# KaranSankla/Lidar_Object_Detection

Measured on AMD Instinct MI355X. Metric: LiDAR points/sec projected+instance-labelled, higher is better.
Workload: dtype f64

## Files before the change

### lidar_object_detection_amd/csrc/lpf_api.hip

```cpp
#include "lpf_kernels.hip.h"
#include "lpf_wide.hip.h"
#include "lpf_cams.hip.h"
#include "lpf_cams_wide.hip.h"
#include "lpf_frame_wide.hip.h"
#include "lpf_depth_maps.hip.h"
#include "lpf_depth_overlays.hip.h"
#include "lpf_match2d.hip.h"
#include "../../include/lpf.h"

#include <algorithm>
#include <cmath>
#include <cstdarg>
#include <cstdio>
#include <cstdlib>
#include <cstring>
#include <dlfcn.h>
#include <mutex>
#include <string>
#include <vector>

#define LPF_SMALL_LAUNCH (7ll << 19)
#define LPF_WIDE_BELOW 480
#define LPF_FEW_BLOCKS 64
#ifndef LPF_TAIL_SPREAD_20THS
#define LPF_TAIL_SPREAD_20THS 13
#endif

#define LPF_RECT_FUSED_TILE 1024

static_assert(sizeof(lpf_frame_summary) == LPF_SUMMARY_BYTES, "summary layout is shared with lpf_finalize_frame");

namespace {

thread_local std::string g_create_error;

struct DevBuf {
    void *p = nullptr;
    size_t cap = 0;
};

}

struct lpf_graph {
    hipGraph_t graph = nullptr;
    hipGraphExec_t exec = nullptr;
    unsigned long long generation = 0;
};

#define LPF_NSETS 4

struct lpf_ctx {
    bool capturing = false;
    unsigned long long generation = 0;
    int device = 0;
    hipStream_t stream = nullptr;
    bool own_stream = false;
    std::string err;

    bool have_camera = false;
    double T[12], K[9], dmin = 0, dmax = 0;
    int W = 0, H = 0;
// ... 174 lines not shown
    const LpfRectJob &GJ = RG ? *RG : norect;
    Y.nrg = RG ? RG->F * RG->bpf : 0;
    Y.nrg8 = (Y.nrg + 7) & ~7;
    Y.ntail = Q.valid ? Q.ntail : 0;
    Y.nk1 = KK.valid ? KK.nk1 : 0;
    Y.npack = 0;
    if (ride) {
        J.masks = (const uint8_t *)c->ride.masks; J.label = c->ride.label; J.M = c->ride.M; J.hw = (long long)c->H * c->W;
        J.rects = c->ride.rects; J.W = c->W;
        J.total16 = (long long)c->ride.F * (J.hw / 16);
        Y.npack = (int)((J.total16 + LPF_BLOCK - 1) / LPF_BLOCK);
    }
    const int nk1_pad = (Y.nk1 + 7) & ~7;
    Y.nper = (Y.ntail + 7) / 8;
    Y.kper = Y.nk1 > 0 ? 8 : 0;
    if (Y.nper > 0 && Y.nk1 > 0) {
        const long long k = ((long long)nk1_pad * LPF_TAIL_SPREAD_20THS / 20 / 8) / Y.nper;
        Y.kper = (int)(k < 1 ? 1 : k) * 8;
    }
    const long long rest = (long long)nk1_pad - (long long)Y.nper * Y.kper;
    Y.rest = (int)(rest > 0 ? rest : 0);
    const long long grid = (long long)Y.nfin8 + Y.nbox8 + Y.nrg8 + (long long)Y.nper * (Y.kper + 8) + Y.rest + Y.npack;
    if (grid > 0) {
        const dim3 gs((unsigned)grid);
        ++c->stats[3];
        if (boxes) ++c->stats[5];
#define LPF_STEP_LAUNCH(RW, LT, PR) do { if (boxes) hipLaunchKernelGGL((lpf_step_t<RW, LPF_K1_FLAGS, LT, PR, true>), gs, dim3(LPF_BLOCK), 0, c->stream, KP, QP, RP, Y, J, XJ, GJ); \
                                         else hipLaunchKernelGGL((lpf_step_t<RW, LPF_K1_FLAGS, LT, PR, false>), gs, dim3(LPF_BLOCK), 0, c->stream, KP, QP, RP, Y, J, XJ, GJ); } while (0)
#define LPF_STEP_LT(RW, PR) do { if (k_lb == 1) LPF_STEP_LAUNCH(RW, uint8_t, PR); else if (k_lb == 2) LPF_STEP_LAUNCH(RW, uint16_t, PR); else LPF_STEP_LAUNCH(RW, uint32_t, PR); } while (0)
        const bool qpre = Q.valid && Q.pre;
        const int rows = KP.tile_pts >> 8;
        if (KK.valid && KK.direct && KK.dsel >= 4) {
            typedef LpfDirectRect<uint8_t, 0> R0; typedef LpfDirectRect<float, 1> R1;
#define LPF_STEP_RECT(RW) do { if (KK.dsel == 4) LPF_STEP_LAUNCH(RW, R0, false); else LPF_STEP_LAUNCH(RW, R1, false); } while (0)
            if (rows == 2) LPF_STEP_RECT(2); else LPF_STEP_RECT(4);
#undef LPF_STEP_RECT
        } else
        if (KK.valid && KK.direct) {
            typedef LpfDirect<uint8_t, 0> D0; typedef LpfDirect<float, 1> D1; typedef LpfDirect<float, 2> D2; typedef LpfDirect<float, 3> D3;
#define LPF_STEP_DIRECT(D) do { if (qpre) LPF_STEP_LAUNCH(2, D, true); else LPF_STEP_LAUNCH(2, D, false); } while (0)
            if (KK.dsel == 0) LPF_STEP_DIRECT(D0); else if (KK.dsel == 1) LPF_STEP_DIRECT(D1); else if (KK.dsel == 2) LPF_STEP_DIRECT(D2); else LPF_STEP_DIRECT(D3);
#undef LPF_STEP_DIRECT
        } else
        if (rows == 2) { if (qpre) LPF_STEP_LT(2, true); else LPF_STEP_LT(2, false); }
        else if (rows == 8) { if (qpre) LPF_STEP_LT(8, true); else LPF_STEP_LT(8, false); }
        else       { if (qpre) LPF_STEP_LT(4, true); else LPF_STEP_LT(4, false); }
#undef LPF_STEP_LT
#undef LPF_STEP_LAUNCH
        LPF_HIP(c, hipGetLastError());
    }
    if (after) LPF_HIP(c, hipEventRecord(after, c->stream));
    if (KK.valid && KK.pre && KK.P.nseg_total > 0) {
        hipLaunchKernelGGL(lpf_scan_segments, dim3(KK.P.F), dim3(LPF_BLOCK), 0, c->stream, KK.P);
        LPF_HIP(c, hipGetLastError());
    }
    return LPF_OK;
}

bool anything_owed(const lpf_ctx *c) { return c->pend_k1.valid || c->pend_tail.valid || c->pend_fin.valid; }

int flush_pending(lpf_ctx *c)
{
    lpf_ctx::BoxSet *XB = &c->bx[c->box_cur];
    if (anything_owed(c)) ++c->stats[1];
    while (anything_owed(c)) {
        const lpf_ctx::Pending K = c->pend_k1, Q = c->pend_tail, R = c->pend_fin;
        int rc_ = launch_step(c, K, Q, R, false, 4, XB, nullptr);
// ... 1027 lines not shown
    NarrowLayout L;
    narrow_layout(c, frame_off, F, BX, out->inst_cap, small, L);
    const bool fused = c->fused && !host_io && pts_on_device && !c->capturing;
    L.split(fused && L.few ? 4 : 1);
    if (c->geometry == 3) L.pre_scan = true;
    if (!fused && anything_owed(c) && (rc = sync_all(c))) return rc;
    lpf_ctx::Scratch &S = c->sc[fused ? c->parity : 0];
    if ((rc = narrow_reserve(c, S, L, M, Btot))) return rc;
    if ((rc = narrow_tables(c, S, L, false))) return rc;
    LpfParams P;
    narrow_params(P, c, ctx_cam(c), L, S, BX, M, out->inst_cap);
    const bool sparse_frames = Ntot * 2 <= (int64_t)F * c->W * c->H;
    const bool direct_rect_fused = c->ride.valid && fused && M > 0 && sparse_frames && !small && c->ride.rects &&
                                   ((!c->ride.f32 && c->ride.mode == 0) || (c->ride.f32 && c->ride.mode == 1));
    const bool direct_fused = direct_rect_fused || (c->ride.valid && fused && small && sparse_frames && M > 0);
    const bool ride_pack = c->ride.valid && fused && !direct_fused && c->ride.can_ride && M > 0;
    if (c->ride.valid && !direct_fused && !ride_pack && (rc = pack_ride_now(c))) return rc;
    const bool direct_rect = M > 0 && c->lazy.valid && !fused && sparse_frames && !small && c->lazy.rects &&
                             ((!c->lazy.f32 && c->lazy.mode == 0) || (c->lazy.f32 && c->lazy.mode == 1));
    const bool direct = direct_rect || (M > 0 && c->lazy.valid && small && sparse_frames && !fused);
    if (M > 0 && c->lazy.valid && !direct && (rc = ensure_packed(c))) return rc;
    const lpf_ctx::Scratch &SM = c->sc[c->mask_set];
    if (M > 0 && fused && !direct && c->mask_set != c->parity)
        return fail(c, LPF_ERR_STATE, "the masks were set for another scratch set: in the pipelined modes the label images rotate with the scratch sets -- call lpf_set_masks_* before every lpf_run* (and after switching modes)");
    P.label_img = (M > 0) ? (direct ? c->lazy.p : direct_fused ? c->ride.masks : SM.label_cur) : nullptr;
    P.rects = (direct && c->lazy.valid) ? c->lazy.rects : (direct_fused && c->ride.valid) ? c->ride.rects : nullptr;
    LpfRectJob RG;
    memset(&RG, 0, sizeof RG);
    const bool rect_tiles = direct_rect || direct_rect_fused;
    if (rect_tiles) {
        RG.rects = P.rects; RG.F = F; RG.M = M;
        RG.cw = (c->W + LPF_RG_CELL - 1) / LPF_RG_CELL; RG.ch = (c->H + LPF_RG_CELL - 1) / LPF_RG_CELL;
        RG.cells = RG.cw * RG.ch; RG.bpf = (RG.cells + LPF_BLOCK - 1) / LPF_BLOCK;
        if ((rc = reserve(c, S.rgrid, (size_t)F * RG.cells * sizeof(uint32_t)))) return rc;
        RG.grid = (uint32_t *)S.rgrid.p;
        P.rect_grid = RG.grid; P.rg_cw = RG.cw; P.rg_cells = RG.cells;
    }
    if (M > 0 && !P.label_img) return fail(c, LPF_ERR_STATE, "no masks for this run's scratch set: in the pipelined modes the label images rotate with the scratch sets -- call lpf_set_masks_* before every lpf_run* (and after switching modes)");

    const size_t n = (size_t)Ntot;
    if (pts_on_device) {
        P.pts = (const float4 *)pts;
    } else {
        if ((rc = reserve(c, c->st_pts, n * 16))) return rc;
        if (n) LPF_HIP(c, hipMemcpyAsync(c->st_pts.p, pts, n * 16, hipMemcpyHostToDevice, c->stream));
        P.pts = (const float4 *)c->st_pts.p;
    }
#define LPF_OUTBUF(field, member, stage, bytes)                                   \
    if (out->member) {                                                            \
        if (host_io) {                                                            \
            if ((rc = reserve(c, c->stage, (bytes)))) return rc;                  \
            P.field = (decltype(P.field))c->stage.p;                              \
        } else {                                                                  \
            P.field = (decltype(P.field))out->member;                             \
        }                                                                         \
    }
    LPF_OUTBUF(uv, uv, st_uv, n * 8)
    LPF_OUTBUF(label_bits, label_bits, st_label, n * 4)
    if (out->uv_valid && !P.uv) { if ((rc = reserve(c, c->st_uv, n * 8))) return rc; P.uv = (decltype(P.uv))c->st_uv.p; }
    if (out->label_valid && !P.label_bits) { if ((rc = reserve(c, c->st_label, n * 4))) return rc; P.label_bits = (decltype(P.label_bits))c->st_label.p; }
    LPF_OUTBUF(uv_valid, uv_valid, st_uvv, n * 8)
    LPF_OUTBUF(label_valid, label_valid, st_labv, n * 4)
    LPF_OUTBUF(depth, depth, st_depth, n * 8)
    LPF_OUTBUF(uf, u_f, st_uf, n * 8)
    LPF_OUTBUF(vf, v_f, st_vf, n * 8)
    LPF_OUTBUF(valid_idx, valid_idx, st_valid, n * 8)
    LPF_OUTBUF(inst_idx, inst_idx, st_inst, (size_t)F * (size_t)out->inst_cap * 8)
    LPF_OUTBUF(count_out, count_mb, st_count, (size_t)(M > 0 ? M : 1) * (Btot > 0 ? Btot : 1) * 4)
    if (host_io || !out->summary) {
// ... 34 lines not shown
            LPF_HIP(c, hipEventCreate(&a));
            LPF_HIP(c, hipEventCreate(&b));
            c->ev.push_back(a); c->ev.push_back(b);
        }
        e0 = c->ev[2 * c->ev_used]; e1 = c->ev[2 * c->ev_used + 1];
        ++c->ev_used;
        LPF_HIP(c, hipEventRecord(e0, c->stream));
    }
    if (fused) {
        lpf_ctx::Pending cur;
        cur.valid = true; cur.P = P; cur.pre = L.pre_scan; cur.ntail = ntail; cur.nk1 = nk1; cur.lb = lb; cur.small = small;
        cur.direct = direct_fused; cur.dsel = direct_rect_fused ? (c->ride.f32 ? 5 : 4) : c->ride.f32 ? c->ride.mode : 0;
        const lpf_ctx::Pending KK = c->defer ? c->pend_k1 : cur, Q = c->pend_tail, R = c->pend_fin;
        if ((rc = launch_step(c, KK, Q, R, ride_pack, lb, &BX, e1, (rect_tiles && c->defer) ? &RG : nullptr))) return rc;
        c->pend_fin = Q;
        c->pend_tail = KK;
        if (c->defer) c->pend_k1 = cur;
        c->ride.valid = false;
        c->parity = (c->parity + 1) % (c->defer ? 4 : 3);
        return LPF_OK;
    }
    if (BX.job_valid && nk1 > 0 && BX.F > 0 && BX.box_off[BX.F] > 0) {
        lpf_ctx::Pending cur, none;
        cur.valid = true; cur.P = P; cur.pre = false; cur.ntail = 0; cur.nk1 = nk1; cur.lb = lb; cur.small = small;
        cur.direct = direct; cur.dsel = direct_rect ? (c->lazy.f32 ? 5 : 4) : c->lazy.f32 ? c->lazy.mode : 0;
        if ((rc = launch_step(c, cur, none, none, false, lb, &BX, e1))) return rc;
    } else {
    if ((rc = launch_box_job(c, BX))) return rc;
    if (nk1 > 0) {
        const dim3 g1((unsigned)nk1);
#define LPF_K1_LAUNCH(R, LT) hipLaunchKernelGGL((lpf_k1_project_t<R, LPF_K1_FLAGS, LT>), g1, dim3(LPF_BLOCK), 0, c->stream, P)
        if (direct_rect) {
            typedef LpfDirectRect<uint8_t, 0> R0; typedef LpfDirectRect<float, 1> R1;
            if (P.tile_pts == 512) { if (!c->lazy.f32) LPF_K1_LAUNCH(2, R0); else LPF_K1_LAUNCH(2, R1); }
            else       { if (!c->lazy.f32) LPF_K1_LAUNCH(4, R0); else LPF_K1_LAUNCH(4, R1); }
        } else if (direct) {
            typedef LpfDirect<uint8_t, 0> D0; typedef LpfDirect<float, 1> D1; typedef LpfDirect<float, 2> D2; typedef LpfDirect<float, 3> D3;
            if (!c->lazy.f32) LPF_K1_LAUNCH(2, D0);
            else if (c->lazy.mode == 1) LPF_K1_LAUNCH(2, D1);
            else if (c->lazy.mode == 2) LPF_K1_LAUNCH(2, D2);
            else LPF_K1_LAUNCH(2, D3);
        } else if (P.tile_pts == 512) { if (lb == 1) LPF_K1_LAUNCH(2, uint8_t); else if (lb == 2) LPF_K1_LAUNCH(2, uint16_t); else LPF_K1_LAUNCH(2, uint32_t); }
        else       { if (lb == 1) LPF_K1_LAUNCH(4, uint8_t); else if (lb == 2) LPF_K1_LAUNCH(4, uint16_t); else LPF_K1_LAUNCH(4, uint32_t); }
#undef LPF_K1_LAUNCH
        LPF_HIP(c, hipGetLastError());
        if (e1) LPF_HIP(c, hipEventRecord(e1, c->stream));
    }
    }
    if (L.pre_scan && L.nseg_total > 0) {
        hipLaunchKernelGGL(lpf_scan_segments, dim3(F), dim3(LPF_BLOCK), 0, c->stream, P);
        LPF_HIP(c, hipGetLastError());
    }
    if (ntail > 0) {
        if (small && P.count_boxes && c->geometry != 4 && (L.nblk <= LPF_WIDE_BELOW || c->geometry == 1)) {
            if (L.pre_scan) hipLaunchKernelGGL((lpf_tail_wide_t<true>), dim3((unsigned)ntail), dim3(64 * LPF_WIDE_WAVES), 0, c->stream, P);
            else hipLaunchKernelGGL((lpf_tail_wide_t<false>), dim3((unsigned)ntail), dim3(64 * LPF_WIDE_WAVES), 0, c->stream, P);
        } else {
            launch_tail(c->stream, P, ntail, L.pre_scan);
        }
        LPF_HIP(c, hipGetLastError());
    }
    hipLaunchKernelGGL(lpf_finalize, dim3(F), dim3(LPF_BLOCK), 0, c->stream, P);
    LPF_HIP(c, hipGetLastError());

    if (host_io) {
        std::vector<lpf_frame_summary> hs((size_t)F);
// ... 1355 lines not shown
```

### lidar_object_detection_amd/csrc/lpf_kernels.hip.h

```cpp
#pragma once
#include <hip/hip_runtime.h>
#include <stdint.h>

#define LPF_BLOCK 256
#define LPF_SEG_QUANTUM 4096
#define LPF_SEG_SMALL 1024
#define LPF_GROUP_SEGS 64
#define LPF_FRM_SHARDS 8
#define LPF_MAX_MASKS_DEV 32
#define LPF_TAB_ROWS 36
#define LPF_TAB_GROUPS 9

struct LpfFrame {
    long long pt_off;
    long long inst_base;
    int N;
    int seg_off;
    int nseg;
    int box_off;
    int B;
    int pad;
    long long cand_off;
    int cand_words;
    int grp_off;
    int shift;
    int pad4;
};

struct LpfParams {
    double T[12];
    double K[9];
    double dmin, dmax;
    int W, H;
    int F, M;
    int seg_pts;
    int nseg_total;
    int nseg_cap;
    int ngrp_cap;
    int oriented;
    long long inst_cap;
    LpfFrame frame0;
    const LpfFrame *frames;
    const LpfFrame *segs;
    const int2 *blks;
    const int4 *cblks;
    int nblk, ncblk;
    int lists_small;
    int csplit;
    const float4 *pts;
    const void *label_img;
    const int4 *rects;
    const uint32_t *rect_grid;
    int rg_cw, rg_cells;
    const double *boxp;
    const float *boxq;
    const unsigned long long *cand;
    int2 *uv;
    uint32_t *label_bits;
    double *depth, *uf, *vf;
    long long *valid_idx;
    int2 *uv_valid;
    uint32_t *label_valid;
    long long *inst_idx;
    int32_t *count_out;
    void *summary;
    unsigned long long *vbal, *mbal;
    uint4 *seg_tab;
    uint4 *grp_tab;
    uint4 *frm_tab;
    uint4 *seg_pre;
    unsigned *cnt;
    float4 *mlist;
    int count_boxes;
    int count_lazy;
    int tile_pts;
};

__device__ __forceinline__ int lpf_lane() { return threadIdx.x & 63; }
__device__ __forceinline__ int lpf_wave() { return threadIdx.x >> 6; }

__device__ __forceinline__ int lpf_xcd_remap(int b, int n)
{
    const int q = n >> 3, r = n & 7, x = b & 7, i = b >> 3;
    return (x < r ? x * (q + 1) : r * (q + 1) + (x - r) * q) + i;
}

// ... 67 lines not shown
                                                      double &uf, double &vf, double &d)
{
    const double x = (double)fx, y = (double)fy, z = (double)fz;
    double cx = TK[0] * x; cx = fma(TK[1], y, cx); cx = fma(TK[2],  z, cx); cx = cx + TK[3];
    double cy = TK[4] * x; cy = fma(TK[5], y, cy); cy = fma(TK[6],  z, cy); cy = cy + TK[7];
    double cz = TK[8] * x; cz = fma(TK[9], y, cz); cz = fma(TK[10], z, cz); cz = cz + TK[11];
    double qx = TK[12] * cx; qx = fma(TK[13], cy, qx); qx = fma(TK[14], cz, qx);
    double qy = TK[15] * cx; qy = fma(TK[16], cy, qy); qy = fma(TK[17], cz, qy);
    d = TK[18] * cx; d = fma(TK[19], cy, d); d = fma(TK[20], cz, d);
    if (d == 0.0) d = -1e-6;
    lpf_div2(qx, qy, fabs(d), uf, vf);
}

__device__ __forceinline__ unsigned lpf_f32_to_u8(float v)
{
    int t;
    if (!(v > -2147483904.0f && v < 2147483648.0f)) t = INT32_MIN; else t = (int)v;
    return (unsigned)t & 0xFFu;
}

template <typename T, int MODE>
__device__ __forceinline__ bool lpf_member(T v)
{
    if (MODE == 0) return v != 0;
    if (MODE == 1) return lpf_f32_to_u8((float)v) != 0u;
    if (MODE == 3) return (float)v > 0.5f;
    return lpf_f32_to_u8((float)v * 255.0f) == 255u;
}

template <typename T, int MODE> struct LpfDirect { };
template <typename LT> struct LpfIsDirect { static constexpr bool value = false; };
template <typename T, int MODE> struct LpfIsDirect<LpfDirect<T, MODE> > { static constexpr bool value = true; };

template <typename T, int MODE> struct LpfDirectRect { };
template <typename LT> struct LpfIsDirectRect { static constexpr bool value = false; };
template <typename T, int MODE> struct LpfIsDirectRect<LpfDirectRect<T, MODE> > { static constexpr bool value = true; };
template <typename T, int MODE> struct LpfIsDirect<LpfDirectRect<T, MODE> > { static constexpr bool value = true; };

template <typename LT>
struct LpfLabelSrc {
    typedef LT elem;
    static __device__ __forceinline__ uint32_t get(const elem *__restrict__ img, const LpfParams &, const int pix, const int4 *, int, int) { return (uint32_t)img[pix]; }
    static __device__ __forceinline__ size_t frame_stride(const LpfParams &P) { return (size_t)P.W * (size_t)P.H; }
};
template <typename T, int MODE>
struct LpfLabelSrc<LpfDirect<T, MODE> > {
    typedef T elem;
    static __device__ __forceinline__ uint32_t get(const elem *__restrict__ msk, const LpfParams &P, const int pix, const int4 *__restrict__ rc,
                                                   const int ui, const int vi)
    {
        const size_t hw = (size_t)P.W * (size_t)P.H;
        uint32_t l = 0;
        for (int m0 = 0; m0 < P.M; m0 += 8) {
            T v[8];
#pragma unroll
            for (int j = 0; j < 8; ++j) v[j] = msk[(size_t)min(m0 + j, P.M - 1) * hw + pix];
#pragma unroll
            for (int j = 0; j < 8; ++j)
                if (m0 + j < P.M && lpf_member<T, MODE>(v[j])) l |= 1u << (m0 + j);
        }
        if (rc && l) {
            uint32_t rest = l;
            while (rest) {
                const int m = __ffs(rest) - 1;
                rest &= rest - 1u;
                const int4 q = rc[m];
                if (!(ui >= q.x && ui < q.z && vi >= q.y && vi < q.w)) l &= ~(1u << m);
            }
        }
        return l;
    }
    static __device__ __forceinline__ size_t frame_stride(const LpfParams &P) { return (size_t)P.M * (size_t)P.W * (size_t)P.H; }
};

template <typename T, int MODE>
struct LpfLabelSrc<LpfDirectRect<T, MODE> > {
    typedef T elem;
    static constexpr int mode = MODE;
    static __device__ __forceinline__ uint32_t get(const elem *__restrict__, const LpfParams &, const int, const int4 *, int, int) { return 0u; }
    static __device__ __forceinline__ size_t frame_stride(const LpfParams &P) { return (size_t)P.M * (size_t)P.W * (size_t)P.H; }
};

#define LPF_F_X4 1u
#define LPF_F_NTLOAD 2u
#define LPF_F_NTSTORE 4u
#define LPF_F_LAB_NOMATH 8u
#define LPF_F_LAB_NOGATHER 16u
#define LPF_F_LAB_NOSTORE 32u

#define LPF_F_LAB_NOBAL 64u
#define LPF_F_LAB_NOTAB 128u

#define LPF_RG_SHIFT 4
#define LPF_RG_CELL (1 << LPF_RG_SHIFT)
__device__ __forceinline__ unsigned lpf_wave_or(unsigned x);

template <int ROWS, unsigned FL, typename LT, bool PRELOADED>
__device__ __forceinline__ void lpf_k1_tile(const LpfParams &P, const int blk, unsigned *s_cnt, float4 (&p)[ROWS])
{
    constexpr int TILE = LPF_BLOCK * ROWS;
    static_assert(LPF_SEG_QUANTUM % TILE == 0 && (LPF_SEG_SMALL % TILE == 0 || ROWS >= 8), "tiles must divide segments (8-row and larger tiles: large geometry only)");
    const int tid = threadIdx.x, lane = lpf_lane(), wave = lpf_wave();
    const int tiles_per_seg = P.seg_pts / TILE;
    const int lb = lpf_xcd_remap(blk, P.nseg_total * tiles_per_seg);
    const int sid = lb / tiles_per_seg;
    LpfFrame fr = P.frame0;
    if (P.F > 1) fr = P.segs[__builtin_amdgcn_readfirstlane(sid)];
    const int f = fr.pad;
    const int sh = fr.shift;
    const long long pbase = fr.pt_off - sh;
    const int seg_start = (sid - fr.seg_off) * P.seg_pts;
    const int seg_end = min(seg_start + P.seg_pts, fr.N + sh);
    const int c = seg_start + (lb - sid * tiles_per_seg) * TILE;
    if (c >= seg_end) return;
    const float4 *__restrict__ pts = P.pts + pbase;
    typedef LpfLabelSrc<LT> Src;
    const typename Src::elem *__restrict__ limg =
        (P.label_img && P.M > 0) ? static_cast<const typename Src::elem *>(P.label_img) + (size_t)f * Src::frame_stride(P) : nullptr;
    const int rows_per_seg = P.seg_pts >> 6;
    if (tid < LPF_TAB_ROWS) s_cnt[tid] = 0;
    __syncthreads();
    unsigned nvalid_w = 0, nmask_w = 0;

    {
        const int wbase = c + wave * (ROWS * 64) + lane;
#pragma unroll
        for (int r = 0; r < ROWS; ++r) {
            if constexpr (PRELOADED) continue;
            const float4 *src = pts + min(wbase + r * 64, seg_end - 1);
            if (FL & LPF_F_NTLOAD) {
                typedef float f4v __attribute__((ext_vector_type(4)));
                const f4v t = __builtin_nontemporal_load(reinterpret_cast<const f4v *>(src));
                p[r] = make_float4(t.x, t.y, t.z, t.w);
            } else {
                p[r] = *src;
            }
        }
        uint32_t lab[ROWS];
        bool valid[ROWS];
        constexpr bool RECT = LpfIsDirectRect<LT>::value;
        const int4 *__restrict__ rc_f = ((RECT || LpfIsDirect<LT>::value) && P.rects) ? P.rects + (size_t)f * P.M : nullptr;
        const uint32_t *__restrict__ rgrid = (RECT && limg && P.rect_grid) ? P.rect_grid + (size_t)f * P.rg_cells : nullptr;
        const size_t mhw = (size_t)P.W * (size_t)P.H;
        unsigned long long myv = 0, mym = 0;
        auto consume = [&](const int r, uint32_t l, const bool okr) {
            const int idx = wbase + r * 64;
            if (idx >= sh && idx < seg_end && P.label_bits && !(FL & LPF_F_LAB_NOSTORE)) {
                if (FL & LPF_F_NTSTORE) __builtin_nontemporal_store(l, P.label_bits + pbase + idx);
                else P.label_bits[pbase + idx] = l;
            }
            const unsigned long long vb = __ballot(okr);
            const unsigned long long mb = __ballot(l != 0);
            if (lane == r) { myv = vb; mym = mb; }
            if (l && P.mlist && !(FL & LPF_F_LAB_NOSTORE))
                P.mlist[pbase + (wbase - lane) + ((wbase - lane) == 0 ? sh : 0) + nmask_w + __popcll(mb & ((1ull << lane) - 1ull))] =
                    make_float4(p[r].x, p[r].y, p[r].z, __uint_as_float(l));
            nvalid_w += __popcll(vb);
            nmask_w += __popcll(mb);
            while (l) {
                const int m = __ffs(l) - 1;
                l &= l - 1;
                atomicAdd(&s_cnt[2 + m], 1u);
            }
        };
#pragma unroll
        for (int r = 0; r < ROWS; ++r) {
            const int idx = wbase + r * 64;
            const bool live = idx >= sh && idx < seg_end;
            if (FL & LPF_F_X4) asm volatile("" ::"v"(p[r].w));
            double uf, vf, d, ru, rv;
            if (FL & LPF_F_LAB_NOMATH) {
                uf = (double)p[r].x; vf = (double)p[r].y; d = (double)p[r].z;
                ru = uf + 700.0; rv = vf + 100.0;
            } else {
                lpf_project_point(P, p[r].x, p[r].y, p[r].z, uf, vf, d);
                ru = rint(uf); rv = rint(vf);
            }
            const int ui = lpf_sat_i32(ru), vi = lpf_sat_i32(rv);
            const bool ok = live && ((unsigned)ui < (unsigned)P.W) && ((unsigned)vi < (unsigned)P.H) &&
                            (d > P.dmin) && (d < P.dmax);
            valid[r] = ok;
            lab[r] = 0;
            if constexpr (RECT) {
                if (ok && rgrid) lab[r] = rgrid[(vi >> LPF_RG_SHIFT) * P.rg_cw + (ui >> LPF_RG_SHIFT)];
            } else
            if (!(FL & LPF_F_LAB_NOGATHER)) {
                if (ok && limg) lab[r] = Src::get(limg, P, vi * P.W + ui, rc_f, ui, vi);
            }
            if (live && !(FL & LPF_F_LAB_NOSTORE)) {
                const long long g = pbase + idx;
                if (P.uv) {
                    if (FL & LPF_F_NTSTORE) {
                        typedef int i2v __attribute__((ext_vector_type(2)));
                        i2v t; t.x = ui; t.y = vi;
                        __builtin_nontemporal_store(t, reinterpret_cast<i2v *>(P.uv + g));
                    } else {
                        P.uv[g] = make_int2(ui, vi);
                    }
                }
                if (P.depth) P.depth[g] = d;
                if (P.uf) P.uf[g] = uf;
                if (P.vf) P.vf[g] = vf;
            }
        }
#pragma unroll
        for (int r = 0; r < ROWS; ++r) {
            uint32_t l = lab[r];
            if constexpr (RECT) {
                if (__any(l != 0u)) {
                    double uf, vf, d;
                    lpf_project_point(P, p[r].x, p[r].y, p[r].z, uf, vf, d);
                    const int ui = lpf_sat_i32(rint(uf)), vi = lpf_sat_i32(rint(vf));
                    const unsigned pix = (unsigned)(vi * P.W + ui);
                    uint32_t any = lpf_wave_or(l), l2 = 0u;
                    while (any) {
                        const int m = __ffs(any) - 1;
                        any &= any - 1u;
                        const int4 q = rc_f[m];
                        const bool in = ((l >> m) & 1u) && ui >= q.x && ui < q.z && vi >= q.y && vi < q.w;
                        if (__any(in)) {
                            const typename Src::elem *__restrict__ mk = limg + (size_t)m * mhw;
                            if (in && lpf_member<typename Src::elem, Src::mode>(mk[pix])) l2 |= 1u << m;
                        }
                    }
                    l = l2;
                }
            }
            consume(r, l, valid[r]);
        }
        if (lane < ROWS && !(FL & LPF_F_LAB_NOBAL)) {
            const size_t row = (size_t)sid * rows_per_seg + ((c - seg_start) >> 6) + wave * ROWS + lane;
            P.vbal[row] = myv;
            P.mbal[row] = mym;
        }
    }
    if (lane == 0) { atomicAdd(&s_cnt[0], nvalid_w); atomicAdd(&s_cnt[1], nmask_w); }
    __syncthreads();
    if (!(FL & LPF_F_LAB_NOTAB)) {
        if (tid < (2 + P.M + 1) >> 1) {
            const unsigned long long v = (unsigned long long)s_cnt[2 * tid] | ((unsigned long long)s_cnt[2 * tid + 1] << 32);
            if (v) {
                int seg_off = P.frame0.seg_off, grp_off = P.frame0.grp_off, fid = P.frame0.pad;
                if (P.F > 1) { const LpfFrame *e = P.segs + lpf_uni(sid); seg_off = e->seg_off; grp_off = e->grp_off; fid = e->pad; }
                const int k = sid - seg_off, g = tid >> 1, h = tid & 1;
                atomicAdd(reinterpret_cast<unsigned long long *>(P.seg_tab + (size_t)g * P.nseg_cap + sid) + h, v);
                atomicAdd(reinterpret_cast<unsigned long long *>(P.grp_tab + (size_t)g * P.ngrp_cap + grp_off + (k >> 6)) + h, v);
                atomicAdd(reinterpret_cast<unsigned long long *>(P.frm_tab + ((size_t)fid * LPF_FRM_SHARDS + (k & (LPF_FRM_SHARDS - 1))) * LPF_TAB_GROUPS + g) + h, v);
            }
        }
    }
}

template <int ROWS, unsigned FL, typename LT>
__device__ __forceinline__ void lpf_k1_tile(const LpfParams &P, const int blk, unsigned *s_cnt)
{
    float4 p[ROWS];
    lpf_k1_tile<ROWS, FL, LT, false>(P, blk, s_cnt, p);
}

template <int ROWS, unsigned FL, typename LT = uint32_t>
__global__ __launch_bounds__(LPF_BLOCK) void lpf_k1_project_t(const LpfParams P)
{
    __shared__ unsigned s_cnt[LPF_TAB_ROWS];
    lpf_k1_tile<ROWS, FL, LT>(P, (int)blockIdx.x, s_cnt);
}

#define LPF_K1_FLAGS (LPF_F_X4 | LPF_F_NTLOAD | LPF_F_NTSTORE)

__device__ __forceinline__ bool lpf_oriented_inside(double px, double py, double pz, const double *__restrict__ b)
{
    const double rx = px - b[0], ry = py - b[1], rz = pz - b[2];
    const bool exact_ok = b[15] != 0.0;
#pragma unroll
    for (int a = 0; a < 3; ++a) {
        const double v0 = b[3 + 4 * a], v1 = b[4 + 4 * a], v2 = b[5 + 4 * a], vv = b[6 + 4 * a];
        double d = v1 * ry; d = fma(v0, rx, d); d = fma(v2, rz, d);
        bool in;
        if (exact_ok && !(fabs(d) < 1e-200 && d != 0.0)) {
            in = (d >= 0.0) && (d <= vv);
        } else {
            const double t = d / vv;
            in = (t >= 0.0) && (t <= 1.0);
        }
        if (!in) return false;
    }
    return true;
}

__device__ __forceinline__ bool lpf_aabb_inside(double px, double py, double pz, const double *__restrict__ b)
{
    return (px >= b[0]) && (px <= b[3]) && (py >= b[1]) && (py <= b[4]) && (pz >= b[2]) && (pz <= b[5]);
}

__device__ __forceinline__ unsigned lpf_rl(unsigned v, int l) { return (unsigned)__builtin_amdgcn_readlane((int)v, l); }
__device__ __forceinline__ float lpf_rlf(float v, int l) { return __int_as_float(__builtin_amdgcn_readlane(__float_as_int(v), l)); }
__device__ __forceinline__ unsigned long long lpf_rl64(unsigned long long v, int l)
{
// ... 636 lines not shown
            w[0] = (long long)tot[0]; w[1] = (long long)tot[1]; w[34] = 0;
            bb[32] = (total > P.inst_cap && P.inst_idx) ? 1 : 0;
            bb[33] = 0;
        }
    }
    if (!staged) {
        __syncthreads();
        for (int i = tid; i < MB; i += LPF_BLOCK) {
            if (out) out[i] = (int32_t)cnt[i];
            cnt[i] = 0;
        }
    }
}

__device__ __forceinline__ int2 lpf_tail_entry(const LpfParams &P, const int i)
{
    if (P.F > 1) return P.blks[i];
    const int first = i * LPF_LISTS_WAVES;
    return make_int2(first, max(0, min(LPF_LISTS_WAVES, P.frame0.nseg - first)));
}
__device__ __forceinline__ void lpf_count_entry(const LpfParams &P, const int i, int &first, int &f, int &nw, int &wd, int &part)
{
    if (P.F > 1) {
        const int4 e = P.cblks[i];
        first = e.x; f = e.y; wd = e.z; nw = e.w & 7; part = e.w >> 3;
        return;
    }
    const int words = max(1, P.frame0.cand_words), per = words * P.csplit;
    const int g = i / per, rem = i - g * per;
    wd = rem / P.csplit; part = rem - wd * P.csplit; f = 0; first = g * LPF_LISTS_WAVES;
    nw = max(0, min(LPF_LISTS_WAVES, P.frame0.nseg - first));
}

struct LpfTailListsLds { unsigned short lidx[LPF_LISTS_WAVES][LPF_LIST_CAP]; };
struct LpfTailCountLds {
    float4 pt[LPF_LISTS_WAVES][64];
    unsigned q[LPF_LISTS_WAVES][128];
    unsigned cnt[LPF_MAX_MASKS_DEV * LPF_BC_WORD / 2];
    float bq[6 * LPF_BC_WORD];
    double bp[LPF_BC_WORD * 16];
    float dom[4];
    unsigned im[LPF_LISTS_WAVES][64], mbase[LPF_LISTS_WAVES][64], L[LPF_LISTS_WAVES];
};

#define LPF_TAIL_LDS (sizeof(LpfTailCountLds) > sizeof(LpfTailListsLds) ? sizeof(LpfTailCountLds) : sizeof(LpfTailListsLds))
#define LPF_STEP_LDS (LPF_TAIL_LDS > sizeof(LpfBoxJobLds) ? LPF_TAIL_LDS : sizeof(LpfBoxJobLds))

template <bool PRE, int STEP>
__device__ __forceinline__ void lpf_tail_block(const LpfParams &P, const int tb, char *s_raw)
{
    LpfTailListsLds &LL = *reinterpret_cast<LpfTailListsLds *>(s_raw);
    LpfTailCountLds &LC = *reinterpret_cast<LpfTailCountLds *>(s_raw);
    const int tid = threadIdx.x, wave = lpf_wave();
    const int ncount = P.count_boxes ? P.ncblk : 0;
    if (tb >= ncount) {
        const int2 ent = lpf_tail_entry(P, tb - ncount);
        const int f = ent.y >> 3, nw = ent.y & 7;
        const LpfFrame fr = lpf_frame_record(P.frame0, P.frames, P.F > 1, f);
        if (wave < nw && (P.valid_idx || P.inst_idx)) {
            if (P.lists_small) lpf_lists_wave_small<PRE>(P, fr, ent.x + wave);
            else lpf_lists_wave<PRE, STEP>(P, fr, ent.x + wave, LL.lidx[wave]);
        }
        return;
    }
    int first, f, nw, wd, part;
    lpf_count_entry(P, tb, first, f, nw, wd, part);
    const LpfFrame fr = lpf_frame_record(P.frame0, P.frames, P.F > 1, f);
    if (wd * LPF_BC_WORD >= fr.B) return;
    if (!P.count_lazy) lpf_count_stage(P, fr, wd, tid, LPF_BLOCK, LC.cnt, LC.bq, LC.bp, LC.dom);
    {
        const int lane = lpf_lane();
        unsigned im = 0, mbase = 0, L = 0;
        if (wave < nw) L = lpf_count_rows(P, fr, first + wave, im, mbase);
        LC.im[wave][lane] = im; LC.mbase[wave][lane] = mbase;
        if (lane == 0) LC.L[wave] = L;
    }
    __syncthreads();
    if (P.count_lazy) {
        if ((LC.L[0] | LC.L[1] | LC.L[2] | LC.L[3]) == 0u) return;
        lpf_count_stage(P, fr, wd, tid, LPF_BLOCK, LC.cnt, LC.bq, LC.bp, LC.dom);
        __syncthreads();
    }
    {
        const int lane = lpf_lane();
        const unsigned L0 = LC.L[0], L1 = LC.L[1], L2 = LC.L[2], L3 = LC.L[3];
        const int c0 = (int)((L0 + 63) >> 6), c1 = (int)((L1 + 63) >> 6), c2 = (int)((L2 + 63) >> 6), c3 = (int)((L3 + 63) >> 6);
        for (int c = part * LPF_LISTS_WAVES + wave; c < c0 + c1 + c2 + c3; c += LPF_LISTS_WAVES * P.csplit) {
            int sg = 0, cc = c;
            if (cc >= c0) { cc -= c0; sg = 1; if (cc >= c1) { cc -= c1; sg = 2; if (cc >= c2) { cc -= c2; sg = 3; } } }
            lpf_count_chunk(P, fr, first + sg, LC.im[sg][lane], LC.mbase[sg][lane], LC.L[sg], (unsigned)cc * 64u, LC.pt[wave], LC.q[wave],
                            LC.cnt, LC.bq, LC.bp, LC.dom, wd);
        }
    }
    __syncthreads();
    lpf_count_flush(P, fr, wd, tid, LPF_BLOCK, LC.cnt);
}

template <bool PRE>
__global__ __launch_bounds__(LPF_BLOCK, 7) void lpf_tail_t(const LpfParams P)
{
// ... 99 lines not shown
    double Tcv[12];
    double K[9];
    int W, H, chunks;
    const LpfBoxFrame *bframes;
    LpfBoxFrame frame0;
    double *boxp; float *boxq; unsigned long long *cand;
    double *corners_keep;
    uint8_t *enabled_out;
    uint8_t *visible; double *corners_out; double *bbox2d; int32_t *front;
};
struct LpfBoxJobLds {
    double c[32][8][3];
    unsigned long long grid[LPF_GRID_CELLS];
    float bnd[64][4];
    float dom[4];
};

__device__ __forceinline__ void lpf_box_frame_block(const LpfBoxJob &J, const int blk, char *s_raw);
struct LpfPackJob {
    const uint8_t *masks;
    void *label;
    long long hw, total16;
    int M, W;
    const int4 *rects;
};
template <typename T, int MODE, typename LT>
__device__ __forceinline__ void lpf_pack16_block(const T *__restrict__ masks, LT *__restrict__ label,
                                                 const int M, const long long hw, const long long total16, const long long blk,
                                                 const int4 *__restrict__ rects, const int W);

struct LpfRectJob {
    const int4 *rects;
    uint32_t *grid;
    int F, M, cw, ch, cells, bpf;
};
__device__ __forceinline__ void lpf_rect_grid_block(const LpfRectJob &G, const int blk)
{
    const int f = blk / G.bpf, i = (blk - f * G.bpf) * LPF_BLOCK + (int)threadIdx.x;
    if (f >= G.F || i >= G.cells) return;
    const int cy = i / G.cw, cx = i - cy * G.cw;
    const int x0 = cx << LPF_RG_SHIFT, y0 = cy << LPF_RG_SHIFT;
    const int4 *__restrict__ rc = G.rects + (size_t)lpf_uni(f) * G.M;
    uint32_t bits = 0u;
    for (int m0 = 0; m0 < G.M; m0 += 8) {
        int4 q[8];
#pragma unroll
        for (int j = 0; j < 8; ++j) q[j] = rc[min(m0 + j, G.M - 1)];
#pragma unroll
        for (int j = 0; j < 8; ++j)
            if (m0 + j < G.M && q[j].x < x0 + LPF_RG_CELL && q[j].z > x0 && q[j].y < y0 + LPF_RG_CELL && q[j].w > y0 && q[j].z > q[j].x && q[j].w > q[j].y)
                bits |= 1u << (m0 + j);
    }
    G.grid[(size_t)f * G.cells + i] = bits;
}
__global__ __launch_bounds__(LPF_BLOCK) void lpf_rect_grid_kernel(const LpfRectJob G) { lpf_rect_grid_block(G, (int)blockIdx.x); }

template <int ROWS, unsigned FL, typename LT, bool PRE, bool BOXES>
__global__ __launch_bounds__(LPF_BLOCK, 7) void lpf_step_t(const LpfParams P, const LpfParams Q, const LpfParams R, const LpfStepLayout Y,
                                                           const LpfPackJob J, const LpfBoxJob X, const LpfRectJob G)
{
    __shared__ __attribute__((aligned(16))) char s_raw[LPF_STEP_LDS];
    __shared__ unsigned s_cnt[LPF_TAB_ROWS];
    int b = (int)blockIdx.x;
    LPF_ROLE_BEGIN
    if (b < Y.nfin8) {
        if (b < Y.nfin) {
            const LpfFrame fr = lpf_frame_record(R.frame0, R.frames, R.F > 1, b);
            lpf_finalize_frame(R, fr, b, s_cnt, reinterpret_cast<unsigned *>(s_raw));
            LPF_ROLE_END(0)
        }
        return;
    }
    b -= Y.nfin8;
    if (b < Y.nbox8) {
        if constexpr (BOXES) {
            if (b < Y.nbox) { lpf_box_frame_block(X, b, s_raw); LPF_ROLE_END(1) }
        }
        return;
    }
    b -= Y.nbox8;
    if (b < Y.nrg8) {
        if (b < Y.nrg) lpf_rect_grid_block(G, b);
        return;
    }
    b -= Y.nrg8;
    const int plen = Y.kper + 8, periodic = Y.nper * plen;
    int vblk;
    if (b < periodic) {
        const int per = b / plen, pos = b - per * plen;
        if (pos >= Y.kper) {
            const int tb = per * 8 + (pos - Y.kper);
            if (tb < Y.ntail) { lpf_tail_block<PRE, 2>(Q, tb, s_raw); LPF_ROLE_END(tb < (Q.count_boxes ? Q.ncblk : 0) ? 3 : 2) }
            return;
        }
        vblk = ((per * (Y.kper >> 3) + (pos >> 3)) << 3) | (pos & 7);
    } else {
        const int r = b - periodic;
        if (r >= Y.rest) {
            if constexpr (!LpfIsDirect<LT>::value) {
                if (r - Y.rest < Y.npack) { lpf_pack16_block<uint8_t, 0, LT>(J.masks, static_cast<LT *>(J.label), J.M, J.hw, J.total16, r - Y.rest, J.rects, J.W); LPF_ROLE_END(4) }
            }
            return;
        }
        vblk = ((Y.nper * (Y.kper >> 3) + (r >> 3)) << 3) | (r & 7);
    }
    const int x = vblk & 7, q = Y.nk1 >> 3, rem = Y.nk1 & 7;
    if ((vblk >> 3) >= q + (x < rem ? 1 : 0)) return;
    lpf_k1_tile<ROWS, FL, LT>(P, vblk, s_cnt);
    LPF_ROLE_END(5)
}

__global__ __launch_bounds__(LPF_BLOCK) void lpf_resize_linear_u8_kernel(const uint8_t *__restrict__ src, uint8_t *__restrict__ dst,
                                                                         const int4 *__restrict__ xtab, const int4 *__restrict__ ytab,
                                                                         const int w, const int h, const int W, const int H, const long long total)
{
    const long long i = (long long)blockIdx.x * LPF_BLOCK + threadIdx.x;
    if (i >= total) return;
    const long long hw = (long long)W * H;
    const long long n = i / hw;
    const int rem = (int)(i - n * hw), y = rem / W, x = rem - y * W;
    const int4 cx = xtab[x], cy = ytab[y];
    const uint8_t *__restrict__ s = src + (size_t)n * w * h;
    const int r0 = cy.x * w, r1 = cy.y * w;
    const int S0 = (int)s[r0 + cx.x] * cx.z + (int)s[r0 + cx.y] * cx.w;
    const int S1 = (int)s[r1 + cx.x] * cx.z + (int)s[r1 + cx.y] * cx.w;
    dst[i] = (uint8_t)((((cy.z * (S0 >> 4)) >> 16) + ((cy.w * (S1 >> 4)) >> 16) + 2) >> 2);
}

#define LPF_R2H_BLOCKS 8
struct LpfToHost {
    long long *valid_idx; int2 *uv_valid; uint32_t *label_valid; long long *inst_idx; int32_t *count_mb; void *summary;
    long long inst_cap;
    int n_count;
};

__global__ __launch_bounds__(LPF_BLOCK) void lpf_results_to_host(const LpfParams P, const LpfToHost D)
{
    const int f = (int)blockIdx.x / LPF_R2H_BLOCKS, part = (int)blockIdx.x - f * LPF_R2H_BLOCKS;
    if (f >= P.F) return;
    const LpfFrame fr = lpf_frame_record(P.frame0, P.frames, P.F > 1, f);
    const long long *S = reinterpret_cast<const long long *>(static_cast<const char *>(P.summary) + (size_t)f * LPF_SUMMARY_BYTES);
// ... 526 lines not shown
```

Before: 173.1 billion.

## Add LDS cell-occupancy bitmap to skip rect-grid gathers; early-exit empty count blocks

```diff
diff --git a/lidar_object_detection_amd/csrc/lpf_api.hip b/lidar_object_detection_amd/csrc/lpf_api.hip
--- a/lidar_object_detection_amd/csrc/lpf_api.hip
+++ b/lidar_object_detection_amd/csrc/lpf_api.hip
@@ -27,6 +27,9 @@
 #endif
 
 #define LPF_RECT_FUSED_TILE 1024
+#ifndef LPF_RECT_LDS
+#define LPF_RECT_LDS 1
+#endif
 
 static_assert(sizeof(lpf_frame_summary) == LPF_SUMMARY_BYTES, "summary layout is shared with lpf_finalize_frame");
 
@@ -267,7 +270,9 @@
         const int rows = KP.tile_pts >> 8;
         if (KK.valid && KK.direct && KK.dsel >= 4) {
             typedef LpfDirectRect<uint8_t, 0> R0; typedef LpfDirectRect<float, 1> R1;
-#define LPF_STEP_RECT(RW) do { if (KK.dsel == 4) LPF_STEP_LAUNCH(RW, R0, false); else LPF_STEP_LAUNCH(RW, R1, false); } while (0)
+            typedef LpfDirectRect<uint8_t, 0, true> R0L; typedef LpfDirectRect<float, 1, true> R1L;
+#define LPF_STEP_RECT(RW) do { if (KP.rg_lds) { if (KK.dsel == 4) LPF_STEP_LAUNCH(RW, R0L, false); else LPF_STEP_LAUNCH(RW, R1L, false); } \
+                               else { if (KK.dsel == 4) LPF_STEP_LAUNCH(RW, R0, false); else LPF_STEP_LAUNCH(RW, R1, false); } } while (0)
             if (rows == 2) LPF_STEP_RECT(2); else LPF_STEP_RECT(4);
 #undef LPF_STEP_RECT
         } else
@@ -1361,9 +1366,14 @@
         RG.rects = P.rects; RG.F = F; RG.M = M;
         RG.cw = (c->W + LPF_RG_CELL - 1) / LPF_RG_CELL; RG.ch = (c->H + LPF_RG_CELL - 1) / LPF_RG_CELL;
         RG.cells = RG.cw * RG.ch; RG.bpf = (RG.cells + LPF_BLOCK - 1) / LPF_BLOCK;
-        if ((rc = reserve(c, S.rgrid, (size_t)F * RG.cells * sizeof(uint32_t)))) return rc;
+        RG.occ_words = (RG.cells + 63) / 64;
+        const size_t grid_bytes = ((size_t)F * RG.cells * sizeof(uint32_t) + 7) & ~(size_t)7;
+        if ((rc = reserve(c, S.rgrid, grid_bytes + (size_t)F * RG.occ_words * sizeof(unsigned long long)))) return rc;
         RG.grid = (uint32_t *)S.rgrid.p;
+        RG.occ = (unsigned long long *)((char *)S.rgrid.p + grid_bytes);
         P.rect_grid = RG.grid; P.rg_cw = RG.cw; P.rg_cells = RG.cells;
+        P.rect_occ = RG.occ; P.rg_occ_words = RG.occ_words;
+        P.rg_lds = (LPF_RECT_LDS && RG.occ_words <= LPF_RG_LDS_WORDS) ? 1 : 0;
     }
     if (M > 0 && !P.label_img) return fail(c, LPF_ERR_STATE, "no masks for this run's scratch set: in the pipelined modes the label images rotate with the scratch sets -- call lpf_set_masks_* before every lpf_run* (and after switching modes)");
 
@@ -1464,6 +1474,11 @@
 #define LPF_K1_LAUNCH(R, LT) hipLaunchKernelGGL((lpf_k1_project_t<R, LPF_K1_FLAGS, LT>), g1, dim3(LPF_BLOCK), 0, c->stream, P)
         if (direct_rect) {
             typedef LpfDirectRect<uint8_t, 0> R0; typedef LpfDirectRect<float, 1> R1;
+            typedef LpfDirectRect<uint8_t, 0, true> R0L; typedef LpfDirectRect<float, 1, true> R1L;
+            if (P.rg_lds) {
+                if (P.tile_pts == 512) { if (!c->lazy.f32) LPF_K1_LAUNCH(2, R0L); else LPF_K1_LAUNCH(2, R1L); }
+                else       { if (!c->lazy.f32) LPF_K1_LAUNCH(4, R0L); else LPF_K1_LAUNCH(4, R1L); }
+            } else
             if (P.tile_pts == 512) { if (!c->lazy.f32) LPF_K1_LAUNCH(2, R0); else LPF_K1_LAUNCH(2, R1); }
             else       { if (!c->lazy.f32) LPF_K1_LAUNCH(4, R0); else LPF_K1_LAUNCH(4, R1); }
         } else if (direct) {
diff --git a/lidar_object_detection_amd/csrc/lpf_kernels.hip.h b/lidar_object_detection_amd/csrc/lpf_kernels.hip.h
--- a/lidar_object_detection_amd/csrc/lpf_kernels.hip.h
+++ b/lidar_object_detection_amd/csrc/lpf_kernels.hip.h
@@ -52,6 +52,9 @@
     const int4 *rects;
     const uint32_t *rect_grid;
     int rg_cw, rg_cells;
+    const unsigned long long *rect_occ;
+    int rg_occ_words;
+    int rg_lds;
     const double *boxp;
     const float *boxq;
     const unsigned long long *cand;
@@ -185,10 +188,10 @@
 template <typename LT> struct LpfIsDirect { static constexpr bool value = false; };
 template <typename T, int MODE> struct LpfIsDirect<LpfDirect<T, MODE> > { static constexpr bool value = true; };
 
-template <typename T, int MODE> struct LpfDirectRect { };
-template <typename LT> struct LpfIsDirectRect { static constexpr bool value = false; };
-template <typename T, int MODE> struct LpfIsDirectRect<LpfDirectRect<T, MODE> > { static constexpr bool value = true; };
-template <typename T, int MODE> struct LpfIsDirect<LpfDirectRect<T, MODE> > { static constexpr bool value = true; };
+template <typename T, int MODE, bool GRID_LDS = false> struct LpfDirectRect { };
+template <typename LT> struct LpfIsDirectRect { static constexpr bool value = false; static constexpr bool grid_lds = false; };
+template <typename T, int MODE, bool G> struct LpfIsDirectRect<LpfDirectRect<T, MODE, G> > { static constexpr bool value = true; static constexpr bool grid_lds = G; };
+template <typename T, int MODE, bool G> struct LpfIsDirect<LpfDirectRect<T, MODE, G> > { static constexpr bool value = true; };
 
 template <typename LT>
 struct LpfLabelSrc {
@@ -226,8 +229,8 @@
     static __device__ __forceinline__ size_t frame_stride(const LpfParams &P) { return (size_t)P.M * (size_t)P.W * (size_t)P.H; }
 };
 
-template <typename T, int MODE>
-struct LpfLabelSrc<LpfDirectRect<T, MODE> > {
+template <typename T, int MODE, bool G>
+struct LpfLabelSrc<LpfDirectRect<T, MODE, G> > {
     typedef T elem;
     static constexpr int mode = MODE;
     static __device__ __forceinline__ uint32_t get(const elem *__restrict__, const LpfParams &, const int, const int4 *, int, int) { return 0u; }
@@ -246,10 +249,11 @@
 
 #define LPF_RG_SHIFT 4
 #define LPF_RG_CELL (1 << LPF_RG_SHIFT)
+#define LPF_RG_LDS_WORDS 512
 __device__ __forceinline__ unsigned lpf_wave_or(unsigned x);
 
 template <int ROWS, unsigned FL, typename LT, bool PRELOADED>
-__device__ __forceinline__ void lpf_k1_tile(const LpfParams &P, const int blk, unsigned *s_cnt, float4 (&p)[ROWS])
+__device__ __forceinline__ void lpf_k1_tile(const LpfParams &P, const int blk, unsigned *s_cnt, float4 (&p)[ROWS], unsigned long long *s_occ = nullptr)
 {
     constexpr int TILE = LPF_BLOCK * ROWS;
     static_assert(LPF_SEG_QUANTUM % TILE == 0 && (LPF_SEG_SMALL % TILE == 0 || ROWS >= 8), "tiles must divide segments (8-row and larger tiles: large geometry only)");
@@ -271,8 +275,10 @@
     const typename Src::elem *__restrict__ limg =
         (P.label_img && P.M > 0) ? static_cast<const typename Src::elem *>(P.label_img) + (size_t)f * Src::frame_stride(P) : nullptr;
     const int rows_per_seg = P.seg_pts >> 6;
+    constexpr bool RECT = LpfIsDirectRect<LT>::value;
+    constexpr bool grid_lds = LpfIsDirectRect<LT>::grid_lds;
     if (tid < LPF_TAB_ROWS) s_cnt[tid] = 0;
-    __syncthreads();
+    if constexpr (!grid_lds) __syncthreads();
     unsigned nvalid_w = 0, nmask_w = 0;
 
     {
@@ -291,7 +297,18 @@
         }
         uint32_t lab[ROWS];
         bool valid[ROWS];
-        constexpr bool RECT = LpfIsDirectRect<LT>::value;
+        const bool have_grid = RECT && limg && P.rect_grid;
+        if constexpr (grid_lds) {
+            unsigned long long t[LPF_RG_LDS_WORDS / LPF_BLOCK];
+            const unsigned long long *__restrict__ occ = P.rect_occ + (size_t)f * P.rg_occ_words;
+#pragma unroll
+            for (int k = 0; k < LPF_RG_LDS_WORDS / LPF_BLOCK; ++k)
+                t[k] = (have_grid && k * LPF_BLOCK + tid < P.rg_occ_words) ? occ[k * LPF_BLOCK + tid] : 0ull;
+#pragma unroll
+            for (int k = 0; k < LPF_RG_LDS_WORDS / LPF_BLOCK; ++k)
+                if (k * LPF_BLOCK < P.rg_occ_words) s_occ[k * LPF_BLOCK + tid] = t[k];
+            __syncthreads();
+        }
         const int4 *__restrict__ rc_f = ((RECT || LpfIsDirect<LT>::value) && P.rects) ? P.rects + (size_t)f * P.M : nullptr;
         const uint32_t *__restrict__ rgrid = (RECT && limg && P.rect_grid) ? P.rect_grid + (size_t)f * P.rg_cells : nullptr;
         const size_t mhw = (size_t)P.W * (size_t)P.H;
@@ -316,6 +333,21 @@
                 atomicAdd(&s_cnt[2 + m], 1u);
             }
         };
+        auto rect_exact = [&](const uint32_t l, const int ui, const int vi) -> uint32_t {
+            const unsigned pix = (unsigned)(vi * P.W + ui);
+            uint32_t any = lpf_wave_or(l), l2 = 0u;
+            while (any) {
+                const int m = __ffs(any) - 1;
+                any &= any - 1u;
+                const int4 q = rc_f[m];
+                const bool in = ((l >> m) & 1u) && ui >= q.x && ui < q.z && vi >= q.y && vi < q.w;
+                if (__any(in)) {
+                    const typename Src::elem *__restrict__ mk = limg + (size_t)m * mhw;
+                    if constexpr (RECT) { if (in && lpf_member<typename Src::elem, Src::mode>(mk[pix])) l2 |= 1u << m; }
+                }
+            }
+            return l2;
+        };
 #pragma unroll
         for (int r = 0; r < ROWS; ++r) {
             const int idx = wbase + r * 64;
@@ -335,7 +367,7 @@
             valid[r] = ok;
             lab[r] = 0;
             if constexpr (RECT) {
-                if (ok && rgrid) lab[r] = rgrid[(vi >> LPF_RG_SHIFT) * P.rg_cw + (ui >> LPF_RG_SHIFT)];
+                if constexpr (!grid_lds) { if (ok && rgrid) lab[r] = rgrid[(vi >> LPF_RG_SHIFT) * P.rg_cw + (ui >> LPF_RG_SHIFT)]; }
             } else
             if (!(FL & LPF_F_LAB_NOGATHER)) {
                 if (ok && limg) lab[r] = Src::get(limg, P, vi * P.W + ui, rc_f, ui, vi);
@@ -355,28 +387,26 @@
                 if (P.uf) P.uf[g] = uf;
                 if (P.vf) P.vf[g] = vf;
             }
+            if constexpr (grid_lds) {
+                const int cell = ok ? (vi >> LPF_RG_SHIFT) * P.rg_cw + (ui >> LPF_RG_SHIFT) : 0;
+                const bool cand = ok && ((s_occ[cell >> 6] >> (cell & 63)) & 1ull);
+                uint32_t l = 0u;
+                if (__any(cand)) {
+                    if (cand) l = rgrid[cell];
+                    if (__any(l != 0u)) l = rect_exact(l, ui, vi);
+                }
+                consume(r, l, ok);
+            }
         }
 #pragma unroll
         for (int r = 0; r < ROWS; ++r) {
+            if constexpr (grid_lds) break;
             uint32_t l = lab[r];
             if constexpr (RECT) {
                 if (__any(l != 0u)) {
                     double uf, vf, d;
                     lpf_project_point(P, p[r].x, p[r].y, p[r].z, uf, vf, d);
-                    const int ui = lpf_sat_i32(rint(uf)), vi = lpf_sat_i32(rint(vf));
-                    const unsigned pix = (unsigned)(vi * P.W + ui);
-                    uint32_t any = lpf_wave_or(l), l2 = 0u;
-                    while (any) {
-                        const int m = __ffs(any) - 1;
-                        any &= any - 1u;
-                        const int4 q = rc_f[m];
-                        const bool in = ((l >> m) & 1u) && ui >= q.x && ui < q.z && vi >= q.y && vi < q.w;
-                        if (__any(in)) {
-                            const typename Src::elem *__restrict__ mk = limg + (size_t)m * mhw;
-                            if (in && lpf_member<typename Src::elem, Src::mode>(mk[pix])) l2 |= 1u << m;
-                        }
-                    }
-                    l = l2;
+                    l = rect_exact(l, lpf_sat_i32(rint(uf)), lpf_sat_i32(rint(vf)));
                 }
             }
             consume(r, l, valid[r]);
@@ -405,17 +435,22 @@
 }
 
 template <int ROWS, unsigned FL, typename LT>
-__device__ __forceinline__ void lpf_k1_tile(const LpfParams &P, const int blk, unsigned *s_cnt)
+__device__ __forceinline__ void lpf_k1_tile(const LpfParams &P, const int blk, unsigned *s_cnt, unsigned long long *s_occ = nullptr)
 {
     float4 p[ROWS];
-    lpf_k1_tile<ROWS, FL, LT, false>(P, blk, s_cnt, p);
+    lpf_k1_tile<ROWS, FL, LT, false>(P, blk, s_cnt, p, s_occ);
 }
 
 template <int ROWS, unsigned FL, typename LT = uint32_t>
 __global__ __launch_bounds__(LPF_BLOCK) void lpf_k1_project_t(const LpfParams P)
 {
     __shared__ unsigned s_cnt[LPF_TAB_ROWS];
-    lpf_k1_tile<ROWS, FL, LT>(P, (int)blockIdx.x, s_cnt);
+    if constexpr (LpfIsDirectRect<LT>::grid_lds) {
+        __shared__ unsigned long long s_occ[LPF_RG_LDS_WORDS];
+        lpf_k1_tile<ROWS, FL, LT>(P, (int)blockIdx.x, s_cnt, s_occ);
+    } else {
+        lpf_k1_tile<ROWS, FL, LT>(P, (int)blockIdx.x, s_cnt);
+    }
 }
 
 #define LPF_K1_FLAGS (LPF_F_X4 | LPF_F_NTLOAD | LPF_F_NTSTORE)
@@ -1118,6 +1153,9 @@
     nw = max(0, min(LPF_LISTS_WAVES, P.frame0.nseg - first));
 }
 
+#ifndef LPF_COUNT_LOOK
+#define LPF_COUNT_LOOK 1
+#endif
 struct LpfTailListsLds { unsigned short lidx[LPF_LISTS_WAVES][LPF_LIST_CAP]; };
 struct LpfTailCountLds {
     float4 pt[LPF_LISTS_WAVES][64];
@@ -1151,7 +1189,18 @@
     }
     int first, f, nw, wd, part;
     lpf_count_entry(P, tb, first, f, nw, wd, part);
+    unsigned masked = 1u;
+    if (LPF_COUNT_LOOK && P.count_lazy) {
+        typedef const __attribute__((address_space(4))) uint4 *LpfConstSeg;
+        const LpfConstSeg st = (LpfConstSeg)(P.seg_tab + lpf_uni(first));
+        masked = 0u;
+        if (nw > 0) {
+#pragma unroll
+            for (int k = 0; k < LPF_LISTS_WAVES; ++k) masked |= st[min(k, nw - 1)].y;
+        }
+    }
     const LpfFrame fr = lpf_frame_record(P.frame0, P.frames, P.F > 1, f);
+    if (lpf_uni((int)masked) == 0) return;
     if (wd * LPF_BC_WORD >= fr.B) return;
     if (!P.count_lazy) lpf_count_stage(P, fr, wd, tid, LPF_BLOCK, LC.cnt, LC.bq, LC.bp, LC.dom);
     {
@@ -1317,7 +1366,9 @@
 struct LpfRectJob {
     const int4 *rects;
     uint32_t *grid;
+    unsigned long long *occ;
     int F, M, cw, ch, cells, bpf;
+    int occ_words;
 };
 __device__ __forceinline__ void lpf_rect_grid_block(const LpfRectJob &G, const int blk)
 {
@@ -1337,6 +1388,8 @@
                 bits |= 1u << (m0 + j);
     }
     G.grid[(size_t)f * G.cells + i] = bits;
+    const unsigned long long any = __ballot(bits != 0u);
+    if ((threadIdx.x & 63) == 0) G.occ[(size_t)f * G.occ_words + (i >> 6)] = any;
 }
 __global__ __launch_bounds__(LPF_BLOCK) void lpf_rect_grid_kernel(const LpfRectJob G) { lpf_rect_grid_block(G, (int)blockIdx.x); }
 
@@ -1391,7 +1444,8 @@
     }
     const int x = vblk & 7, q = Y.nk1 >> 3, rem = Y.nk1 & 7;
     if ((vblk >> 3) >= q + (x < rem ? 1 : 0)) return;
-    lpf_k1_tile<ROWS, FL, LT>(P, vblk, s_cnt);
+    static_assert(LPF_STEP_LDS >= LPF_RG_LDS_WORDS * sizeof(unsigned long long), "the tiles' occupancy bits live in the roles' LDS");
+    lpf_k1_tile<ROWS, FL, LT>(P, vblk, s_cnt, LpfIsDirectRect<LT>::grid_lds ? reinterpret_cast<unsigned long long *>(s_raw) : nullptr);
     LPF_ROLE_END(5)
 }
 
```

After: 171.9 billion, median of 2. About the same (-0.7%).
